# JuliaMeshless/WhatsThePoint.jl

Measured on AMD Instinct MI355X. Metric: Mpoints/sec per repel iter (k=21 KNN+force), higher is better.
Workload: dtype f32

## Files before the change

### include/wtp.h

```cpp
#ifndef WTP_H
#define WTP_H

#include <stdint.h>

#ifdef __cplusplus
extern "C" {
#endif

typedef struct wtp_ctx wtp_ctx;

typedef enum wtp_status {
    WTP_OK = 0,
    WTP_ERR_ARG = 1,
    WTP_ERR_OOM = 2,
    WTP_ERR_HIP = 3,
    WTP_ERR_STATE = 4,
    WTP_ERR_NO_DEVICE = 5
} wtp_status;

typedef enum wtp_dtype { WTP_F32 = 0, WTP_F64 = 1 } wtp_dtype;

typedef enum wtp_force_kind {
    WTP_FORCE_INVERSE_DISTANCE = 0,
    WTP_FORCE_SPACING_EQUILIBRIUM = 1,
// ... 190 lines not shown
                             double r, int64_t* d_offsets_out, wtp_block_topo_info* info);
int wtp_block_radius_fill(wtp_ctx* ctx, int64_t* d_idx_out);
int wtp_comm_exchange_peers(wtp_ctx* ctx, int n_msgs, const int* peers, const void* const* d_send, const int64_t* n_send,
                            void* const* d_recv, const int64_t* n_recv);
int wtp_comm_allgather_dev(wtp_ctx* ctx, const void* d_send, void* d_recv, int64_t bytes);

int wtp_relax_set_coverage(wtp_ctx* ctx, int axis, double lo, double hi);
int wtp_relax_set_coverage_box(wtp_ctx* ctx, const double lo[3], const double hi[3]);

int wtp_relax_set_fixed_dev(wtp_ctx* ctx, const void* d_fixed4, int64_t n_fixed_new);


int wtp_timers_get(wtp_ctx* ctx, double out[4]);
int wtp_timers_reset(wtp_ctx* ctx);
int wtp_debug_diag(wtp_ctx* ctx, unsigned long long out[16]);

int wtp_gen_uniform_dev(wtp_ctx* ctx, uint64_t seed, int64_t first, int64_t n, int dim, int dtype,
                        void* d_out);

#ifdef __cplusplus
}
#endif
#endif
```

### whatsthepoint.jl_amd/_lib.py

```python
from __future__ import annotations

import ctypes as C
import os
import subprocess

_HERE = os.path.dirname(os.path.abspath(__file__))
CSRC = os.path.join(_HERE, "csrc")
SO_PATH = os.environ.get("WTP_LIB") or os.path.join(CSRC, "libwtp.so")

WTP_OK, WTP_ERR_ARG, WTP_ERR_OOM, WTP_ERR_HIP, WTP_ERR_STATE, WTP_ERR_NO_DEVICE = range(6)
WTP_F32, WTP_F64 = 0, 1
WTP_SPACING_CONSTANT, WTP_SPACING_PER_POINT, WTP_SPACING_LOGLIKE, WTP_SPACING_BOUNDARY_LAYER = range(4)


class WtpError(RuntimeError):

    def __init__(self, code, msg):
        super().__init__(f"libwtp status {code}: {msg}")
        self.code = code


class WtpArgumentError(ValueError):
    """WTP_ERR_ARG: the reference throws ArgumentError for the same input (src/repel.jl:74)."""

# ... 102 lines not shown
    "wtp_block_step": (_i, [_vp, C.POINTER(StepStats), C.POINTER(BlockInfo)]),
    "wtp_block_run": (_i, [_vp, _i, _vp, C.POINTER(StepStats), C.POINTER(BlockInfo)]),
    "wtp_block_run_until": (_i, [_vp, _i, _d, _i, _d, _vp, C.POINTER(_i), C.POINTER(_i), C.POINTER(StepStats)]),
    "wtp_block_get": (_i, [_vp, _vp, _vp, _i64, C.POINTER(_i64)]),
    "wtp_block_close": (_i, [_vp]),
    "wtp_block_grid": (_i, [_i, C.POINTER(_i)]),
    "wtp_block_morton_rank": (_i, [_i, _i, _i, C.POINTER(_i)]),
    "wtp_block_knn": (_i, [_vp, _i, _i, _vp, _vp, _i64, _i, _i, _d, _vp, _vp, C.POINTER(BlockTopoInfo)]),
    "wtp_block_radius_offsets": (_i, [_vp, _i, _i, _vp, _vp, _i64, _d, _vp, C.POINTER(BlockTopoInfo)]),
    "wtp_block_radius_fill": (_i, [_vp, _vp]),
    "wtp_comm_exchange_peers": (_i, [_vp, _i, C.POINTER(_i), C.POINTER(_vp), C.POINTER(_i64), C.POINTER(_vp), C.POINTER(_i64)]),
    "wtp_comm_allgather_dev": (_i, [_vp, _vp, _vp, _i64]),
    "wtp_timers_get": (_i, [_vp, C.POINTER(_d)]),
    "wtp_timers_reset": (_i, [_vp]),
    "wtp_debug_diag": (_i, [_vp, C.POINTER(C.c_ulonglong)]),
    "wtp_gen_uniform_dev": (_i, [_vp, C.c_uint64, _i64, _i64, _i, _i, _vp]),
}

_lib = None


def build(verbose: bool = False) -> str:
    res = subprocess.run(["make", "-C", CSRC, "-j4"], capture_output=True, text=True)
    if res.returncode != 0:
        raise RuntimeError("building libwtp.so failed:\n" + res.stdout[-4000:] + res.stderr[-4000:])
    if verbose:
        print(res.stdout[-2000:])
    return SO_PATH


# ... 31 lines not shown
```

### whatsthepoint.jl_amd/csrc/wtp_api.hip

```cpp
#include <cmath>
#include <cstdlib>
#include <cstring>
#include <type_traits>

#include "wtp_internal.hpp"

namespace wtp {

static thread_local std::string g_create_err;

int fail(wtp_ctx* ctx, int code, const std::string& msg) {
    if (ctx)
        ctx->err = msg;
    else
        g_create_err = msg;
    return code;
}

int ensure(wtp_ctx* ctx, DevBuf& b, size_t bytes) {
    if (bytes == 0) bytes = 16;
    if (b.cap >= bytes) return WTP_OK;
    if (b.p) {
        hipFree(b.p);
        b.p = nullptr;
// ... 1172 lines not shown
    const double cell_f = (cs2 && r.spacing_kind == WTP_SPACING_CONSTANT) ? 1.01 : 1.1;
    return {cs2 ? kRhoCs2 : 3.5 * (ctx->rho / 9.0),
            cell_f * r.force.u0 * (r.spacing_typ < r.spacing_max ? r.spacing_typ : r.spacing_max)};
}

static SweepRoute step_route(const RelaxState& r, bool fresh) {
    if (!fresh) return route_ball(r.route) ? SweepRoute::Ball : SweepRoute::Exact;
    const bool measured = r.route == SweepRoute::Ksel ? r.tune.bx > 0 : !route_cs(r.route) || r.brick_hcap > 0;
    if (measured) return r.route;
    return r.route == SweepRoute::Cs64 || r.route == SweepRoute::Cs64Wave ? SweepRoute::Exact : SweepRoute::Select;
}

static int ball_pass(wtp_ctx* ctx, SearchArgs<float>& a) { return launch_cs_ball(ctx, a, a.ball_list, a.ball_count); }
static int ball_pass(wtp_ctx* ctx, SearchArgs<double>& a) { return launch_cs_ball64(ctx, a, a.ball_list, a.ball_count); }

template <typename T> static int launch_sweep(wtp_ctx* ctx, SearchArgs<T>& a, SweepRoute route, bool ball) {
    constexpr bool f32 = sizeof(T) == 4;
    ctx->n_sweep_launches += 1;
    int rc = WTP_OK, sp = -1;
    switch (route) {
    case SweepRoute::Exact:
    case SweepRoute::Ball:
        sp = span_begin(ctx, 1);
        if (route == SweepRoute::Ball) {
            rc = launch_cs_all_slots(ctx, a.fb_list, a.n, a.fb_count);
            if (!rc) rc = ball_pass(ctx, a);
        }
        if (!rc) rc = launch_generic_sweep<T>(ctx, a, route == SweepRoute::Exact);
        span_end(ctx, sp);
        return rc;
    case SweepRoute::F64Ksel:
        if constexpr (!f32) rc = relax_f64_ksel_sweep(ctx, a, &sp);
        break;
    case SweepRoute::Ksel:
        sp = span_begin(ctx, 1);
        if constexpr (f32) rc = launch_ksel_sweep(ctx, a);
        a.fb_r0 = 3;
        break;
    case SweepRoute::Select:
    case SweepRoute::Cs:
    case SweepRoute::Cs2:
        sp = span_begin(ctx, 1);
        if constexpr (f32) {
// ... 11 lines not shown
    case SweepRoute::Cs64Wave:
        sp = span_begin(ctx, 1);
        if constexpr (!f32) {
            rc = launch_brick_cs<double>(ctx, a);
            if (!rc && ball) rc = ball_pass(ctx, a);
        }
        break;
    }
    span_end(ctx, sp);
    if (rc) return rc;
    sp = span_begin(ctx, 2);
    if constexpr (f32) {
        if (route == SweepRoute::Cs2) rc = launch_cs2_followup(ctx, a);
        if (!rc && ball) rc = ball_pass(ctx, a);
    }
    if (!rc) rc = launch_generic_sweep<T>(ctx, a, false);
    span_end(ctx, sp);
    return rc;
}

template <typename T>
static HashBuild<T> relax_request(const wtp_ctx* ctx, const RelaxState& r, const Pt<T>* in, Pt<T>* out, int64_t n, int k,
                                  const HashView& view, bool keep_grid) {
    const RouteGrid g = route_grid(ctx, r);
    HashBuild<T> b(in, out, n, r.dim, k);
    b.rho_direct = g.rho;
    b.min_cell = g.min_cell;
    b.cell_scale = r.tune.scale;
    b.view = view;
    b.keep_grid = keep_grid;
    b.canonical = !r.tune.valid || r.route != SweepRoute::F64Ksel;
// ... 127 lines not shown
        a.cap_count = (float)(4.18879 * kGammaCapSweep * kGammaCapSweep * kGammaCapSweep * ctx->rho * (a.k + 1) / 22.0);
    }
    if (route == SweepRoute::Cs64 || route == SweepRoute::Cs64Wave) a.gamma_cap = (T)kGammaCap;
    a.tnn_frac = (T)kTnnFrac;
    a.cover_axis = r.cover_axis;
    a.cover_lo = (T)r.cover_lo;
    a.cover_hi = (T)r.cover_hi;
    for (int ax = 0; ax < 3; ++ax) {
        a.cover_lo3[ax] = (T)r.cover_lo3[ax];
        a.cover_hi3[ax] = (T)r.cover_hi3[ax];
    }
    a.uncovered = (int32_t*)ctx->fb_count.p + 8;
    if (!ctx->counters_clean) WTP_HIP(ctx, hipMemsetAsync(ctx->fb_count.p, 0, 64, ctx->stream));
    ctx->counters_clean = false;
    a.used_brick = a.used_wave = a.used_generic = 0;
    if ((rc = launch_sweep<T>(ctx, a, route, ball && route_ball(route)))) return rc;
    int sp = span_begin(ctx, 2);
    if (r.wall_active) {
        char* wf = (char*)ctx->wall_flags.p;
        rc = launch_mesh_constrain<T>(ctx, a.query, a.out, r.n, r.n_fixed, r.wall_offset, (const uint8_t*)wf,
                                      (uint8_t*)wf + r.wall_nm, (int32_t*)ctx->wall_tri.p, (int32_t*)ctx->wall_hint.p,
                                      (int32_t*)ctx->fb_count.p + 12);
        if (rc) return rc;
    }
    rc = launch_reduce_partials(ctx, a.partials, a.n_partials, a.used_brick, a.used_wave, a.used_generic, a.fb_count,
                                a.uncovered, r.wall_active ? (const int32_t*)ctx->fb_count.p + 12 : nullptr, d_slot);
    span_end(ctx, sp);
    if (rc) return rc;
    r.bufOld = r.bufP;
    r.bufP = o;
    r.can_revert = true;
    r.have_point_data = true;
    r.sweeps_since_rebuild += 1;
    return WTP_OK;
}

static int relax_step_any(wtp_ctx* ctx, int rebuild, wtp_step_stats* d_slot) {
    return by_dtype(ctx->relax.dtype, [&](auto t) { return relax_step_t<decltype(t)>(ctx, rebuild, d_slot); });
}
int wtp::relax_step_enqueue(wtp_ctx* ctx, int rebuild, wtp_step_stats* d_slot) { return relax_step_any(ctx, rebuild, d_slot); }

int wtp::relax_prerank(wtp_ctx* ctx, int64_t n_fixed_new) {
    RelaxState& r = ctx->relax;
// ... 722 lines not shown
    out[2] = ctx->t_other;
    out[3] = (double)ctx->n_sweep_launches;
    return WTP_OK;
}

WTP_API int wtp_timers_reset(wtp_ctx* ctx) {
    if (!ctx) return WTP_ERR_ARG;
    hipSetDevice(ctx->device);
    spans_collect(ctx);
    ctx->t_hash = ctx->t_sweep = ctx->t_other = 0;
    ctx->n_sweep_launches = 0;
    if (!ctx->timing_forced) ctx->timing = true;
    return WTP_OK;
}

WTP_API int wtp_debug_diag(wtp_ctx* ctx, unsigned long long out[16]) {
    if (!ctx || !out) return WTP_ERR_ARG;
    WTP_HIP(ctx, hipSetDevice(ctx->device));
    int rc;
    if ((rc = ensure(ctx, ctx->diag, 128))) return rc;
    WTP_HIP(ctx, hipMemcpyAsync(out, ctx->diag.p, 128, hipMemcpyDeviceToHost, ctx->stream));
    WTP_HIP(ctx, hipMemsetAsync(ctx->diag.p, 0, 128, ctx->stream));
    if ((rc = sync(ctx))) return rc;
    if (ctx->debug_kd) {
        unsigned long long kd[2] = {0, 0};
        wtp::debug_kd_steps(kd);
        fprintf(stderr, "[wtp] kd walk: %llu node visits by %llu wave-walks (%.1f per walk)\n", kd[0], kd[1], kd[1] ? (double)kd[0] / (double)kd[1] : 0.0);
    }
    return WTP_OK;
}
// ... 11 lines not shown
```

### whatsthepoint.jl_amd/csrc/wtp_device.hpp

```cpp
#pragma once
#include "wtp_internal.hpp"

namespace wtp {

template <typename T> struct Lim;
template <> struct Lim<float> {
    static __device__ __host__ constexpr float inf() { return __builtin_huge_valf(); }
};
template <> struct Lim<double> {
    static __device__ __host__ constexpr double inf() { return __builtin_huge_val(); }
};

__device__ inline float wsqrt(float x) { return __builtin_sqrtf(x); }
__device__ inline double wsqrt(double x) { return __builtin_sqrt(x); }
__device__ inline float wfloor(float x) { return floorf(x); }
__device__ inline double wfloor(double x) { return floor(x); }
__device__ inline float wpow(float a, float b) { return powf(a, b); }
__device__ inline double wpow(double a, double b) { return pow(a, b); }

template <typename T>
__device__ inline T dist2(T ax, T ay, T az, T bx, T by, T bz) {
    T dx = ax - bx;
    T dy = ay - by;
    T dz = az - bz;
// ... 182 lines not shown
    a.sum_u2 += b.sum_u2;
    a.n_move += b.n_move;
    if (b.argmin_i >= 0 &&
        (a.argmin_i < 0 || b.argmin_r < a.argmin_r || (b.argmin_r == a.argmin_r && b.argmin_i < a.argmin_i))) {
        a.argmin_r = b.argmin_r;
        a.argmin_i = b.argmin_i;
        a.argmin_j = b.argmin_j;
    }
}

__device__ inline double shfl_down_d(double v, int d) { return __shfl_down(v, d, 64); }
__device__ inline int64_t shfl_down_i64(int64_t v, int d) {
    return (int64_t)__shfl_down((long long)v, d, 64);
}

__device__ inline void acc_block_reduce(Acc& acc, Acc* smem) {
#pragma unroll
    for (int d = 32; d >= 1; d >>= 1) {
        Acc o;
        o.max_force = shfl_down_d(acc.max_force, d);
        o.sum_u = shfl_down_d(acc.sum_u, d);
        o.sum_u2 = shfl_down_d(acc.sum_u2, d);
        o.argmin_r = shfl_down_d(acc.argmin_r, d);
        o.argmin_i = shfl_down_i64(acc.argmin_i, d);
        o.argmin_j = shfl_down_i64(acc.argmin_j, d);
        o.n_move = shfl_down_i64(acc.n_move, d);
        acc_merge(acc, o);
    }
    int lane = threadIdx.x & 63, wave = threadIdx.x >> 6;
    if (lane == 0) smem[wave] = acc;
    __syncthreads();
    if (threadIdx.x == 0) {
        int nw = (blockDim.x + 63) >> 6;
        for (int w = 1; w < nw; ++w) acc_merge(acc, smem[w]);
    }
}

__device__ inline void acc_store(Partial* p, const Acc& acc) {
    p->max_force = acc.max_force;
    p->sum_u = acc.sum_u;
    p->sum_u2 = acc.sum_u2;
    p->argmin_r = acc.argmin_r;
    p->argmin_i = acc.argmin_i;
    p->argmin_j = acc.argmin_j;
    p->n_move = acc.n_move;
}

__device__ inline void reduce_partials_block(const Partial* __restrict__ parts, int n_parts, int used_brick, int wave_base,
                                             int used_wave, int used_generic, const int32_t* __restrict__ fb_count,
                                             const int32_t* __restrict__ uncovered, const int32_t* __restrict__ escaped,
                                             wtp_step_stats* __restrict__ out, int32_t* __restrict__ counters, Acc* sm) {
    Acc acc = acc_empty();
    const int total = used_brick + used_wave + used_generic;
    for (int t = threadIdx.x; t < total; t += blockDim.x) {
        const int i = t < used_brick ? t
                                     : (t < used_brick + used_wave ? wave_base + (t - used_brick)
                                                                   : n_parts - kGenericPartials + (t - used_brick - used_wave));
        if (parts[i].n_move == 0) continue;
        Acc o;
        o.max_force = parts[i].max_force;
        o.sum_u = parts[i].sum_u;
        o.sum_u2 = parts[i].sum_u2;
        o.argmin_r = parts[i].argmin_r;
        o.argmin_i = parts[i].argmin_i;
        o.argmin_j = parts[i].argmin_j;
        o.n_move = parts[i].n_move;
        acc_merge(acc, o);
    }
    acc_block_reduce(acc, sm);
    if (threadIdx.x == 0) {
        out->max_force = acc.max_force;
        out->sum_u = acc.sum_u;
        out->sum_u2 = acc.sum_u2;
        out->n_move = acc.n_move;
        out->argmin_i = acc.argmin_i;
        out->argmin_j = acc.argmin_j;
        out->argmin_r = acc.argmin_r;
        out->n_fallback = fb_count ? *fb_count : 0;
        out->n_uncovered = uncovered ? *uncovered : 0;
        out->n_escaped = escaped ? *escaped : 0;
    }
    __syncthreads();
    if (counters && threadIdx.x < 16) counters[threadIdx.x] = 0;
}


typedef float f4 __attribute__((ext_vector_type(4)));

__device__ inline uint32_t f2u(float f) { return __builtin_bit_cast(uint32_t, f); }
__device__ inline float u2f(uint32_t u) { return __builtin_bit_cast(float, u); }

__device__ inline float4 lds_pt(const void* base, uint32_t byte_off) {
    return *reinterpret_cast<const float4*>(reinterpret_cast<const unsigned char*>(base) + byte_off);
}

__device__ inline void lds_read_group(f4 (&c)[4], uint32_t addr) {
    asm volatile(
        "ds_read_b128 %0, %4\n\t"
// ... 33 lines not shown
```

### whatsthepoint.jl_amd/csrc/wtp_generic.hip

```cpp
#include "wtp_device.hpp"

namespace wtp {

static constexpr int kThreads = 128;

template <typename T, int MODE>
__global__ __launch_bounds__(kThreads) void generic_kernel(SearchArgs<T> a, const int32_t* __restrict__ list,
                                                           const int32_t* __restrict__ list_count,
                                                           int all, int part_base) {
    if (a.stop && *a.stop) return;
    __shared__ Acc sm_acc[kThreads / 64];
    const Grid<T> g = *a.grid;
    const int nq = all ? a.n : *list_count;
    const int K = a.k;
    const bool skip_self = (MODE == 0) && !a.include_self;
    T bd[kGenericKMax];
    int32_t bi[kGenericKMax];
    int32_t bp[kGenericKMax];
    Acc acc = acc_empty();

    for (int qi = blockIdx.x * blockDim.x + threadIdx.x; qi < nq; qi += gridDim.x * blockDim.x) {
        const int slot = all ? qi : list[qi];
        const Pt<T> q = a.query[slot];
        const int32_t id = w_to_id(q.w);
        if (MODE == 1 && id < a.n_fixed) {
            a.out[slot] = q;
            a.forces[slot] = (T)0;
            a.nn_dist[slot] = Lim<T>::inf();
            a.nn_id[slot] = -1;
            continue;
        }
        const int cx = cell_coord(g, q.x, 0), cy = cell_coord(g, q.y, 1), cz = cell_coord(g, q.z, 2);
        int m = 0;
        for (int r = 1;; r *= 2) {
            m = 0;
            const int z0 = cz - r < 0 ? 0 : cz - r, z1 = cz + r > g.n[2] - 1 ? g.n[2] - 1 : cz + r;
// ... 48 lines not shown
                add_force<T>(a, g.dim, s, q.x, q.y, q.z, id, c.x, c.y, c.z, bi[j], bd[j], Fx, Fy, Fz);
            }
            Pt<T> o;
            const T f = step_point<T>(a, s, q.x, q.y, q.z, Fx, Fy, Fz, o.x, o.y, o.z);
            o.w = q.w;
            a.out[slot] = o;
            a.forces[slot] = f;
            a.nn_dist[slot] = nd;
            a.nn_id[slot] = nid;
            acc_point<T>(acc, f, nd, s, id, nid);
            const T need = m == K ? bd[K - 1] : Lim<T>::inf();
            if (reaches_past_cover<T>(a, q.x, q.y, q.z, need)) atomicAdd(a.uncovered, 1);
        }
    }
    if (MODE == 1) {
        acc_block_reduce(acc, sm_acc);
        if (threadIdx.x == 0) acc_store(&a.partials[part_base + blockIdx.x], acc);
    }
}

template <typename T>
__global__ void pack_queries_kernel(const T* __restrict__ xyz, int64_t nq, int dim, Pt<T>* __restrict__ out) {
    const int64_t i = (int64_t)blockIdx.x * blockDim.x + threadIdx.x;
    if (i >= nq) return;
    Pt<T> p;
    p.x = xyz[i * dim];
    p.y = xyz[i * dim + 1];
    p.z = dim == 3 ? xyz[i * dim + 2] : (T)0;
    p.w = id_to_w((T)0, (int32_t)i);
    out[i] = p;
}

template <typename T> int launch_query_knn(wtp_ctx* ctx, SearchArgs<T>& a, const T* d_xyz, int dim, Pt<T>* d_packed) {
    hipLaunchKernelGGL(pack_queries_kernel<T>, dim3((unsigned)((a.n + 255) / 256)), dim3(256), 0, ctx->stream, d_xyz,
                       (int64_t)a.n, dim, d_packed);
    a.query = d_packed;
    a.include_self = 1;
    hipLaunchKernelGGL((generic_kernel<T, 0>), dim3(grid_for(a.n, kThreads, 4096)), dim3(kThreads), 0, ctx->stream, a,
                       (const int32_t*)nullptr, (const int32_t*)nullptr, 1, 0);
    WTP_HIP(ctx, hipGetLastError());
    return WTP_OK;
}

template <typename T>
__global__ __launch_bounds__(kThreads) void radius_kernel(SearchArgs<T> a, T r, const int64_t* __restrict__ offsets,
                                                          int32_t* __restrict__ idx_out, T* __restrict__ d2_tmp,
                                                          const int32_t* __restrict__ list,
                                                          const int32_t* __restrict__ list_count) {
    const Grid<T> g = *a.grid;
    const T r2 = r * r;
    const int nq = list ? *list_count : a.n;
    for (int qi = blockIdx.x * blockDim.x + threadIdx.x; qi < nq; qi += gridDim.x * blockDim.x) {
        const int slot = list ? list[qi] : qi;
        const Pt<T> q = a.snap[slot];
// ... 24 lines not shown
                    }
                    d2_tmp[base + pos] = d;
                    idx_out[base + pos] = cid;
                    ++m;
                }
            }
    }
}


template <typename T> int launch_generic_topology(wtp_ctx* ctx, SearchArgs<T>& a, bool all) {
    if (!a.counters_cleared) WTP_HIP(ctx, hipMemsetAsync(a.fb2_count, 0, sizeof(int32_t), ctx->stream));
    int rc = launch_wave_topology<T>(ctx, a, all);
    if (rc) return rc;
    hipLaunchKernelGGL((generic_kernel<T, 0>), dim3(256), dim3(kThreads), 0, ctx->stream, a, a.fb2_list,
                       a.fb2_count, 0, 0);
    WTP_HIP(ctx, hipGetLastError());
    return WTP_OK;
}


template <typename T> int launch_generic_sweep(wtp_ctx* ctx, SearchArgs<T>& a, bool all) {
    const int part_base = a.n_partials - kGenericPartials;
    int rc = launch_wave_sweep<T>(ctx, a, all);
    if (rc) return rc;
    a.used_generic = grid_for(a.n / 16, kThreads, 256);
    hipLaunchKernelGGL((generic_kernel<T, 1>), dim3(a.used_generic), dim3(kThreads), 0, ctx->stream, a, a.fb2_list,
                       a.fb2_count, 0, part_base);
    WTP_HIP(ctx, hipGetLastError());
    return WTP_OK;
}

template <typename T> static bool brick_radius_usable(wtp_ctx*, SearchArgs<T>&) { return false; }
template <> bool brick_radius_usable<float>(wtp_ctx* ctx, SearchArgs<float>& a) {
    return !ctx->force_generic && a.fb_list != nullptr && a.fb_count != nullptr;
}
template <typename T> static int brick_radius(wtp_ctx*, SearchArgs<T>&) { return WTP_OK; }
template <> int brick_radius<float>(wtp_ctx* ctx, SearchArgs<float>& a) { return launch_brick_radius(ctx, a); }

__global__ void radius_copy_rows_kernel(int64_t n, const int32_t* __restrict__ tmp, const uint8_t* __restrict__ done,
                                        const int32_t* __restrict__ arena, const int64_t* __restrict__ arena_off,
                                        const int64_t* __restrict__ offsets, int32_t* __restrict__ idx) {
    const int64_t grp = ((int64_t)blockIdx.x * blockDim.x + threadIdx.x) >> 4, ngrp = ((int64_t)gridDim.x * blockDim.x) >> 4;
// ... 67 lines not shown
    int rc;
    if ((brick_radius_usable<T>(ctx, a) && a.rad_tmp) || a.rad_dense)
        rc = launch_wave_radius_fill<T>(ctx, a, r, d_offsets, d_idx, a.fb_list, a.fb_count);
    else
        rc = launch_wave_radius_fill<T>(ctx, a, r, d_offsets, d_idx, nullptr, nullptr);
    if (rc) return rc;
    hipLaunchKernelGGL((radius_kernel<T>), dim3(256), dim3(kThreads), 0, ctx->stream, a, r, d_offsets, d_idx,
                       (T*)ctx->scratch.p, (const int32_t*)a.fb2_list, (const int32_t*)a.fb2_count);
    WTP_HIP(ctx, hipGetLastError());
    return WTP_OK;
}

#define INST(T)                                                                              \
    template int launch_generic_topology<T>(wtp_ctx*, SearchArgs<T>&, bool);                 \
    template int launch_query_knn<T>(wtp_ctx*, SearchArgs<T>&, const T*, int, Pt<T>*);         \
    template int launch_generic_sweep<T>(wtp_ctx*, SearchArgs<T>&, bool);                    \
    template int launch_radius_count<T>(wtp_ctx*, SearchArgs<T>&, T, int32_t*);              \
    template int launch_radius_fill<T>(wtp_ctx*, SearchArgs<T>&, T, const int64_t*, int32_t*);
INST(float)
INST(double)
#undef INST

}
```

### whatsthepoint.jl_amd/csrc/wtp_hash.hip

```cpp
#include "wtp_device.hpp"

namespace wtp {

static constexpr int kThreads = 256;

template <typename T>
__global__ void load_points_kernel(const T* __restrict__ xyz, Pt<T>* __restrict__ out, int64_t n, int dim) {
    int64_t i = (int64_t)blockIdx.x * blockDim.x + threadIdx.x;
    int64_t stride = (int64_t)gridDim.x * blockDim.x;
    for (; i < n; i += stride) {
        Pt<T> p;
        p.x = xyz[i * dim + 0];
        p.y = xyz[i * dim + 1];
        p.z = dim == 3 ? xyz[i * dim + 2] : (T)0;
        p.w = id_to_w((T)0, (int32_t)i);
        out[i] = p;
    }
}

template <typename T>
__global__ void bbox_kernel(const Pt<T>* __restrict__ pts, int64_t n, T* __restrict__ part, int64_t v_old = 0,
                            int32_t v_fixed_old = 0) {
    __shared__ T sm[6][kThreads / 64];
    T mn[3] = {Lim<T>::inf(), Lim<T>::inf(), Lim<T>::inf()};
// ... 798 lines not shown
    for (; i < n; i += stride)
        for (int a = 0; a < dim; ++a) {
            uint64_t h = splitmix64((seed << 40) + 3ull * (uint64_t)(first + i) + (uint64_t)a);
            out[i * dim + a] = (T)((float)(h >> 40) * (1.0f / 16777216.0f));
        }
}

template <typename T>
int launch_gen_uniform(wtp_ctx* ctx, uint64_t seed, int64_t first, int64_t n, int dim, T* d_out) {
    hipLaunchKernelGGL(gen_uniform_kernel<T>, dim3(grid_for(n, kThreads, 8192)), dim3(kThreads), 0,
                       ctx->stream, seed, first, n, dim, d_out);
    WTP_HIP(ctx, hipGetLastError());
    return WTP_OK;
}

__global__ void reduce_partials_kernel(const Partial* __restrict__ parts, int n_parts, int used_brick, int wave_base,
                                       int used_wave, int used_generic, const int32_t* __restrict__ fb_count,
                                       const int32_t* __restrict__ uncovered, const int32_t* __restrict__ escaped,
                                       wtp_step_stats* __restrict__ out, int32_t* __restrict__ counters) {
    __shared__ Acc sm[kThreads / 64];
    reduce_partials_block(parts, n_parts, used_brick, wave_base, used_wave, used_generic, fb_count, uncovered, escaped, out,
                          counters, sm);
}

int launch_reduce_partials(wtp_ctx* ctx, const Partial* parts, int n_parts, int used_brick, int used_wave,
                           int used_generic, const int32_t* fb_count, const int32_t* uncovered, const int32_t* escaped,
                           wtp_step_stats* d_slot) {
    hipLaunchKernelGGL(reduce_partials_kernel, dim3(1), dim3(kThreads), 0, ctx->stream, parts, n_parts, used_brick,
                       brick_partials(), used_wave, used_generic, fb_count, uncovered, escaped, d_slot,
                       (int32_t*)ctx->fb_count.p);
    ctx->counters_clean = true;
    WTP_HIP(ctx, hipGetLastError());
    return WTP_OK;
}

static constexpr int kLayerPasses = 32;
static constexpr int kLayerChunk = kThreads * kLayerPasses;

int layer_blocks(int64_t n) { return (int)((n + kLayerChunk - 1) / kLayerChunk); }

template <typename T> __device__ inline T axis_of(const Pt<T>& p, int axis) {
    return axis == 0 ? p.x : (axis == 1 ? p.y : p.z);
}

__device__ inline int64_t layer_slot(int block, int wave, int pass, int lane) {
// ... 253 lines not shown
```

### whatsthepoint.jl_amd/csrc/wtp_internal.hpp

```cpp
#pragma once
#include <hip/hip_runtime.h>
#include <stdint.h>
#include <map>
#include <string>
#include <utility>
#include <vector>

#include "../../include/wtp.h"

namespace wtp {

template <typename T> struct PtOf;
template <> struct PtOf<float> { using type = float4; };
template <> struct PtOf<double> { using type = double4; };
template <typename T> using Pt = typename PtOf<T>::type;

template <typename F> inline auto by_dtype(int dtype, F&& f) { return dtype == WTP_F32 ? f(float{}) : f(double{}); }

__host__ __device__ inline float id_to_w(float, int32_t id) { return __builtin_bit_cast(float, id); }
__host__ __device__ inline double id_to_w(double, int32_t id) {
    return __builtin_bit_cast(double, (int64_t)id);
}
__host__ __device__ inline int32_t w_to_id(float w) { return __builtin_bit_cast(int32_t, w); }
__host__ __device__ inline int32_t w_to_id(double w) {
// ... 31 lines not shown
constexpr double kGammaCapSweep = 0.96;
constexpr double kTnnFrac = 0.8;
constexpr double kRhoCs2 = 1.0;
constexpr double kRhoKsel = 1.2;
constexpr double kCapKsel = 40.0;
constexpr int kGridReuseMax = 7;

struct Partial {
    double max_force;
    double sum_u;
    double sum_u2;
    double argmin_r;
    int64_t argmin_i;
    int64_t argmin_j;
    int64_t n_move;
};

struct ForceParams {
    int32_t kind;
    double beta, u0, gamma;
};

template <typename T> struct SearchArgs {
    const Grid<T>* grid;
    const Pt<T>* snap;
    const int32_t* cell_start;
    const Pt<T>* query;
    int32_t n;
    int32_t k;
    int32_t include_self;
// ... 191 lines not shown
    size_t cs2_smem = 0;
    const void* cs2_fn = nullptr;
    int cs2_occ = 0;
    std::map<std::pair<const void*, size_t>, int> launch_cache;
    wtp::GridTune knn_tune, knn64_tune;
    wtp::DevBuf pts[3];
    wtp::DevBuf raw_in;
    wtp::DevBuf cell_of, rank_of, cell_cnt, cell_start, scan_tmp;
    wtp::DevBuf grid, bbox_part, occ;
    wtp::DevBuf box_dev;
    wtp::DevBuf idx_out, dist_out, counts_out;
    wtp::DevBuf cand_idx, cand_dist, f32_pts;
    wtp::DevBuf grid_b, cell_start_b, box_b, f64k_s64, f64k_slot, f64k_lists, f64k_cnt;
    wtp::DevBuf forces, nn_dist, nn_id, spacing_pp;
    wtp::DevBuf partials, stats, fb_list, fb_count, fb2_list, fb2_count, nn_list;
    wtp::DevBuf rad_pos;
    wtp::DevBuf rad_bricks;
    bool rad_dense_attr[2] = {false, false};
    bool rad_dense_used = false;
    wtp::DevBuf rad_tmp, rad_done;
    wtp::DevBuf rad_arena, rad_arena_off;
    wtp::DevBuf brick_dead;
    wtp::Prerank prerank;
    int64_t preranked_builds = 0;
    hipStream_t comm_stream = nullptr;
    hipEvent_t ev_comm_a = nullptr, ev_comm_b = nullptr;
    bool hash_scratch_clean = false;
    bool counters_clean = false;
    wtp::DevBuf stop_state;
    const int32_t* stop_dev = nullptr;
// ... 83 lines not shown
    return (int)(b > cap ? cap : b);
}
template <typename T> int launch_topology(wtp_ctx* ctx, SearchArgs<T>& a);
int launch_brick_sweep(wtp_ctx* ctx, SearchArgs<float>& a, bool cs);
template <typename T> int launch_brick_cs(wtp_ctx* ctx, SearchArgs<T>& a);
template <typename T> int launch_wave_topology(wtp_ctx* ctx, SearchArgs<T>& a, bool all);
template <typename T> int launch_wave_sweep(wtp_ctx* ctx, SearchArgs<T>& a, bool all);
template <typename T>
int launch_wave_radius_count(wtp_ctx* ctx, SearchArgs<T>& a, T r, int32_t* d_counts, const int32_t* list,
                             const int32_t* list_count);
template <typename T>
int launch_wave_radius_fill(wtp_ctx* ctx, SearchArgs<T>& a, T r, const int64_t* d_offsets, int32_t* d_idx,
                            const int32_t* list, const int32_t* list_count);
template <typename T> int launch_generic_topology(wtp_ctx* ctx, SearchArgs<T>& a, bool all);
template <typename T> int launch_query_knn(wtp_ctx* ctx, SearchArgs<T>& a, const T* d_xyz, int dim, Pt<T>* d_packed);
template <typename T> int launch_generic_sweep(wtp_ctx* ctx, SearchArgs<T>& a, bool all);
inline int total_partials() { return brick_partials() + kWavePartials + kGenericPartials; }
int launch_brick_radius(wtp_ctx* ctx, SearchArgs<float>& a);
int launch_cs2(wtp_ctx* ctx, SearchArgs<float>& a);
int launch_cs2_followup(wtp_ctx* ctx, SearchArgs<float>& a);
int debug_kd_steps(unsigned long long out[2]);
int launch_cs_ball(wtp_ctx* ctx, SearchArgs<float>& a, int32_t* rest_list, int32_t* rest_count);
int launch_cs2_census(wtp_ctx* ctx, int BX, unsigned int* d_out513);
int launch_cs2_dead(wtp_ctx* ctx, SearchArgs<float>& a, uint8_t* d_dead, int dead_cap);
int cs2_max_bx();
int launch_ksel_topology(wtp_ctx* ctx, SearchArgs<float>& a);
int launch_ksel_sweep(wtp_ctx* ctx, SearchArgs<float>& a);
int ksel_max_bx();
int ksel_kmax();
template <typename T>
int launch_radius_count(wtp_ctx* ctx, SearchArgs<T>& a, T r, int32_t* d_counts);
template <typename T>
int launch_radius_fill(wtp_ctx* ctx, SearchArgs<T>& a, T r, const int64_t* d_offsets,
                       int32_t* d_idx);
int launch_reduce_partials(wtp_ctx* ctx, const Partial* parts, int n_parts, int used_brick, int used_wave,
                           int used_generic, const int32_t* fb_count, const int32_t* uncovered,
                           const int32_t* escaped, wtp_step_stats* d_stats_slot);
template <typename T>
int launch_pca_normals(wtp_ctx* ctx, const T* d_xyz, int64_t n, int dim, const int32_t* d_rows, int k, T* d_out);
template <typename T>
int launch_minplus_batch(wtp_ctx* ctx, const int32_t* d_rows, const T* d_dist, int64_t n, int k, double g, double tol,
                         T* d_h0, T* d_h1, int first, int sweeps, unsigned long long* d_state);
template <typename TP>
int launch_mesh_constrain(wtp_ctx* ctx, const Pt<TP>* old, Pt<TP>* cur, int64_t n, int64_t n_fixed, double offset,
                          const uint8_t* is_bnd, uint8_t* escaped, int32_t* tri_idx, int32_t* hint, int32_t* n_escaped);
template <typename T>
int launch_unpermute(wtp_ctx* ctx, const Pt<T>* pts, int64_t n, int64_t n_fixed, int dim, T* d_xyz_out);
template <typename T>
int launch_unpermute_point_data(wtp_ctx* ctx, const Pt<T>* pts, int64_t n, int64_t n_fixed,
                                const T* forces, const T* nn_dist, const int32_t* nn_id,
                                T* forces_o, T* nn_dist_o, int32_t* nn_id_o);
template <typename T>
// ... 67 lines not shown
```

### whatsthepoint.jl_amd/csrc/wtp_wave.hip

```cpp
#include "wtp_device.hpp"

namespace wtp {

static constexpr int kWaves = 4;
static constexpr int kThreads = kWaves * 64;
static constexpr int kCap = 512;
static constexpr int kKeyRegs = kCap / 64;
static constexpr int kSurv = 256;

template <typename T> struct Bits;
template <> struct Bits<float> {
    using U = uint32_t;
    static __device__ U of(float v) { return __builtin_bit_cast(uint32_t, v); }
    static __device__ float back(U u) { return __builtin_bit_cast(float, u); }
    static constexpr U kInf = 0x7F800000u;
};
template <> struct Bits<double> {
    using U = uint64_t;
    static __device__ U of(double v) { return __builtin_bit_cast(uint64_t, v); }
    static __device__ double back(U u) { return __builtin_bit_cast(double, u); }
    static constexpr U kInf = 0x7FF0000000000000ull;
};

template <typename T, bool SWEEP> struct WaveSmem;
// ... 22 lines not shown

template <typename T, int MODE>
__global__ __launch_bounds__(kThreads) void wave_kernel(SearchArgs<T> a, const int32_t* __restrict__ list,
                                                        const int32_t* __restrict__ list_count, int all,
                                                        int part_base) {
    if (a.stop && *a.stop) return;
    extern __shared__ __attribute__((aligned(16))) unsigned char smem_raw[];
    using U = typename Bits<T>::U;
    const int wave = threadIdx.x >> 6;
    const int lane = threadIdx.x & 63;
    using Smem = WaveSmem<T, MODE == 1>;
    Smem* sm = reinterpret_cast<Smem*>(smem_raw) + wave;
    Acc* sm_acc = reinterpret_cast<Acc*>(smem_raw + sizeof(Smem) * kWaves);
    const Grid<T> g = *a.grid;
    const int nq = all ? a.n : *list_count;
    const int K = a.k;
    const bool skip_self = (MODE == 0) && !a.include_self;
    Acc acc = acc_empty();
    const int wave_global = blockIdx.x * kWaves + wave;
    const int wave_stride = gridDim.x * kWaves;

    for (int qi = wave_global; qi < nq; qi += wave_stride) {
        const int slot = all ? qi : list[qi];
        const Pt<T> q = a.query[slot];
        const int32_t id = w_to_id(q.w);
        if (MODE == 1 && id < a.n_fixed) {
            if (lane == 0) {
                a.out[slot] = q;
                a.forces[slot] = (T)0;
                a.nn_dist[slot] = Lim<T>::inf();
// ... 491 lines not shown
```

Measured before the change: 12510.

## Fuse step-stat reduction into generic sweep kernel via last-block completion

```diff
diff --git a/include/wtp.h b/include/wtp.h
--- a/include/wtp.h
+++ b/include/wtp.h
@@ -228,6 +228,7 @@
 int wtp_timers_get(wtp_ctx* ctx, double out[4]);
 int wtp_timers_reset(wtp_ctx* ctx);
 int wtp_debug_diag(wtp_ctx* ctx, unsigned long long out[16]);
+int wtp_debug_counters(wtp_ctx* ctx, int32_t out[16]);
 
 int wtp_gen_uniform_dev(wtp_ctx* ctx, uint64_t seed, int64_t first, int64_t n, int dim, int dtype,
                         void* d_out);
diff --git a/whatsthepoint.jl_amd/_lib.py b/whatsthepoint.jl_amd/_lib.py
--- a/whatsthepoint.jl_amd/_lib.py
+++ b/whatsthepoint.jl_amd/_lib.py
@@ -140,6 +140,7 @@
     "wtp_timers_get": (_i, [_vp, C.POINTER(_d)]),
     "wtp_timers_reset": (_i, [_vp]),
     "wtp_debug_diag": (_i, [_vp, C.POINTER(C.c_ulonglong)]),
+    "wtp_debug_counters": (_i, [_vp, C.POINTER(C.c_int32)]),
     "wtp_gen_uniform_dev": (_i, [_vp, C.c_uint64, _i64, _i64, _i, _i, _vp]),
 }
 
diff --git a/whatsthepoint.jl_amd/csrc/wtp_api.hip b/whatsthepoint.jl_amd/csrc/wtp_api.hip
--- a/whatsthepoint.jl_amd/csrc/wtp_api.hip
+++ b/whatsthepoint.jl_amd/csrc/wtp_api.hip
@@ -1210,7 +1210,7 @@
 static int ball_pass(wtp_ctx* ctx, SearchArgs<float>& a) { return launch_cs_ball(ctx, a, a.ball_list, a.ball_count); }
 static int ball_pass(wtp_ctx* ctx, SearchArgs<double>& a) { return launch_cs_ball64(ctx, a, a.ball_list, a.ball_count); }
 
-template <typename T> static int launch_sweep(wtp_ctx* ctx, SearchArgs<T>& a, SweepRoute route, bool ball) {
+template <typename T> static int launch_sweep(wtp_ctx* ctx, SearchArgs<T>& a, SweepRoute route, bool ball, StepReduce* red) {
     constexpr bool f32 = sizeof(T) == 4;
     ctx->n_sweep_launches += 1;
     int rc = WTP_OK, sp = -1;
@@ -1222,7 +1222,7 @@
             rc = launch_cs_all_slots(ctx, a.fb_list, a.n, a.fb_count);
             if (!rc) rc = ball_pass(ctx, a);
         }
-        if (!rc) rc = launch_generic_sweep<T>(ctx, a, route == SweepRoute::Exact);
+        if (!rc) rc = launch_generic_sweep<T>(ctx, a, route == SweepRoute::Exact, red);
         span_end(ctx, sp);
         return rc;
     case SweepRoute::F64Ksel:
@@ -1264,7 +1264,7 @@
         if (route == SweepRoute::Cs2) rc = launch_cs2_followup(ctx, a);
         if (!rc && ball) rc = ball_pass(ctx, a);
     }
-    if (!rc) rc = launch_generic_sweep<T>(ctx, a, false);
+    if (!rc) rc = launch_generic_sweep<T>(ctx, a, false, red);
     span_end(ctx, sp);
     return rc;
 }
@@ -1422,19 +1422,30 @@
     if (!ctx->counters_clean) WTP_HIP(ctx, hipMemsetAsync(ctx->fb_count.p, 0, 64, ctx->stream));
     ctx->counters_clean = false;
     a.used_brick = a.used_wave = a.used_generic = 0;
-    if ((rc = launch_sweep<T>(ctx, a, route, ball && route_ball(route)))) return rc;
-    int sp = span_begin(ctx, 2);
+    if ((rc = ensure(ctx, ctx->last_counters, 64))) return rc;
+    StepReduce red{};
+    red.parts = a.partials;
+    red.n_parts = a.n_partials;
+    red.wave_base = brick_partials();
+    red.uncovered = a.uncovered;
+    red.counters = (int32_t*)ctx->fb_count.p;
+    red.last_counters = (int32_t*)ctx->last_counters.p;
+    red.out = r.wall_active ? nullptr : d_slot;
+    if ((rc = launch_sweep<T>(ctx, a, route, ball && route_ball(route), &red))) return rc;
     if (r.wall_active) {
+        int sp = span_begin(ctx, 2);
         char* wf = (char*)ctx->wall_flags.p;
         rc = launch_mesh_constrain<T>(ctx, a.query, a.out, r.n, r.n_fixed, r.wall_offset, (const uint8_t*)wf,
                                       (uint8_t*)wf + r.wall_nm, (int32_t*)ctx->wall_tri.p, (int32_t*)ctx->wall_hint.p,
                                       (int32_t*)ctx->fb_count.p + 12);
         if (rc) return rc;
-    }
-    rc = launch_reduce_partials(ctx, a.partials, a.n_partials, a.used_brick, a.used_wave, a.used_generic, a.fb_count,
-                                a.uncovered, r.wall_active ? (const int32_t*)ctx->fb_count.p + 12 : nullptr, d_slot);
-    span_end(ctx, sp);
-    if (rc) return rc;
+        red.escaped = (const int32_t*)ctx->fb_count.p + 12;
+        red.out = d_slot;
+        rc = launch_reduce_partials(ctx, red);
+        span_end(ctx, sp);
+        if (rc) return rc;
+    }
+    ctx->counters_clean = true;
     r.bufOld = r.bufP;
     r.bufP = o;
     r.can_revert = true;
@@ -2187,6 +2198,16 @@
     return WTP_OK;
 }
 
+WTP_API int wtp_debug_counters(wtp_ctx* ctx, int32_t out[16]) {
+    if (!ctx || !out) return WTP_ERR_ARG;
+    WTP_HIP(ctx, hipSetDevice(ctx->device));
+    int rc;
+    if ((rc = sync(ctx))) return rc;
+    memset(out, 0, 16 * sizeof(int32_t));
+    if (ctx->last_counters.p) WTP_HIP(ctx, hipMemcpy(out, ctx->last_counters.p, 16 * sizeof(int32_t), hipMemcpyDeviceToHost));
+    return WTP_OK;
+}
+
 WTP_API int wtp_debug_diag(wtp_ctx* ctx, unsigned long long out[16]) {
     if (!ctx || !out) return WTP_ERR_ARG;
     WTP_HIP(ctx, hipSetDevice(ctx->device));
diff --git a/whatsthepoint.jl_amd/csrc/wtp_device.hpp b/whatsthepoint.jl_amd/csrc/wtp_device.hpp
--- a/whatsthepoint.jl_amd/csrc/wtp_device.hpp
+++ b/whatsthepoint.jl_amd/csrc/wtp_device.hpp
@@ -220,7 +220,7 @@
     return (int64_t)__shfl_down((long long)v, d, 64);
 }
 
-__device__ inline void acc_block_reduce(Acc& acc, Acc* smem) {
+__device__ inline void acc_wave_reduce(Acc& acc) {
 #pragma unroll
     for (int d = 32; d >= 1; d >>= 1) {
         Acc o;
@@ -233,6 +233,9 @@
         o.n_move = shfl_down_i64(acc.n_move, d);
         acc_merge(acc, o);
     }
+}
+__device__ inline void acc_block_reduce(Acc& acc, Acc* smem) {
+    acc_wave_reduce(acc);
     int lane = threadIdx.x & 63, wave = threadIdx.x >> 6;
     if (lane == 0) smem[wave] = acc;
     __syncthreads();
@@ -252,29 +255,54 @@
     p->n_move = acc.n_move;
 }
 
-__device__ inline void reduce_partials_block(const Partial* __restrict__ parts, int n_parts, int used_brick, int wave_base,
-                                             int used_wave, int used_generic, const int32_t* __restrict__ fb_count,
-                                             const int32_t* __restrict__ uncovered, const int32_t* __restrict__ escaped,
-                                             wtp_step_stats* __restrict__ out, int32_t* __restrict__ counters, Acc* sm) {
-    Acc acc = acc_empty();
-    const int total = used_brick + used_wave + used_generic;
-    for (int t = threadIdx.x; t < total; t += blockDim.x) {
-        const int i = t < used_brick ? t
-                                     : (t < used_brick + used_wave ? wave_base + (t - used_brick)
-                                                                   : n_parts - kGenericPartials + (t - used_brick - used_wave));
-        if (parts[i].n_move == 0) continue;
-        Acc o;
-        o.max_force = parts[i].max_force;
-        o.sum_u = parts[i].sum_u;
-        o.sum_u2 = parts[i].sum_u2;
-        o.argmin_r = parts[i].argmin_r;
-        o.argmin_i = parts[i].argmin_i;
-        o.argmin_j = parts[i].argmin_j;
-        o.n_move = parts[i].n_move;
-        acc_merge(acc, o);
-    }
-    acc_block_reduce(acc, sm);
+constexpr int kReduceThreads = 256;
+template <int NT> __device__ inline void reduce_partials_block(const StepReduce& r, Acc* sm ) {
+    static_assert(kReduceThreads % NT == 0 && NT % 64 == 0, "the block must tile the reduction's threads in whole waves");
+    constexpr int V = kReduceThreads / NT;
+    const int nw = r.wave_count ? (__hip_atomic_load(r.wave_count, __ATOMIC_RELAXED, __HIP_MEMORY_SCOPE_AGENT) +
+                                   kWaveQueriesPerBlock - 1) / kWaveQueriesPerBlock
+                                : r.used_wave;
+    const int ng = r.generic_count ? (__hip_atomic_load(r.generic_count, __ATOMIC_RELAXED, __HIP_MEMORY_SCOPE_AGENT) +
+                                      kGenericQueriesPerBlock - 1) / kGenericQueriesPerBlock
+                                   : r.used_generic;
+    const int used_wave = nw < r.used_wave ? nw : r.used_wave, used_generic = ng < r.used_generic ? ng : r.used_generic;
+    const int total = r.used_brick + used_wave + used_generic;
+#pragma unroll
+    for (int v = 0; v < V; ++v) {
+        Acc acc = acc_empty();
+        for (int t0 = threadIdx.x + v * NT; t0 < total; t0 += 4 * kReduceThreads) {
+            Partial q[4];
+#pragma unroll
+            for (int u = 0; u < 4; ++u) {
+                const int t = t0 + u * kReduceThreads;
+                const int i = t < r.used_brick ? t
+                                               : (t < r.used_brick + used_wave ? r.wave_base + (t - r.used_brick)
+                                                                                 : r.n_parts - kGenericPartials + (t - r.used_brick - used_wave));
+                if (t < total) q[u] = r.parts[i];
+                else q[u].n_move = 0;
+            }
+#pragma unroll
+            for (int u = 0; u < 4; ++u) {
+                if (q[u].n_move == 0) continue;
+                Acc o;
+                o.max_force = q[u].max_force;
+                o.sum_u = q[u].sum_u;
+                o.sum_u2 = q[u].sum_u2;
+                o.argmin_r = q[u].argmin_r;
+                o.argmin_i = q[u].argmin_i;
+                o.argmin_j = q[u].argmin_j;
+                o.n_move = q[u].n_move;
+                acc_merge(acc, o);
+            }
+        }
+        acc_wave_reduce(acc);
+        if ((threadIdx.x & 63) == 0) sm[(threadIdx.x + v * NT) >> 6] = acc;
+    }
+    __syncthreads();
     if (threadIdx.x == 0) {
+        Acc acc = sm[0];
+        for (int w = 1; w < kReduceThreads / 64; ++w) acc_merge(acc, sm[w]);
+        wtp_step_stats* out = r.out;
         out->max_force = acc.max_force;
         out->sum_u = acc.sum_u;
         out->sum_u2 = acc.sum_u2;
@@ -282,12 +310,31 @@
         out->argmin_i = acc.argmin_i;
         out->argmin_j = acc.argmin_j;
         out->argmin_r = acc.argmin_r;
-        out->n_fallback = fb_count ? *fb_count : 0;
-        out->n_uncovered = uncovered ? *uncovered : 0;
-        out->n_escaped = escaped ? *escaped : 0;
-    }
-    __syncthreads();
-    if (counters && threadIdx.x < 16) counters[threadIdx.x] = 0;
+        out->n_fallback = r.fb_count ? __hip_atomic_load(r.fb_count, __ATOMIC_RELAXED, __HIP_MEMORY_SCOPE_AGENT) : 0;
+        out->n_uncovered = r.uncovered ? __hip_atomic_load(r.uncovered, __ATOMIC_RELAXED, __HIP_MEMORY_SCOPE_AGENT) : 0;
+        out->n_escaped = r.escaped ? __hip_atomic_load(r.escaped, __ATOMIC_RELAXED, __HIP_MEMORY_SCOPE_AGENT) : 0;
+    }
+    __syncthreads();
+    if (r.counters && threadIdx.x < 16) {
+        const int32_t c = __hip_atomic_load(r.counters + threadIdx.x, __ATOMIC_RELAXED, __HIP_MEMORY_SCOPE_AGENT);
+        if (r.last_counters) r.last_counters[threadIdx.x] = c;
+        r.counters[threadIdx.x] = 0;
+    }
+}
+
+template <int NT> __device__ inline void finish_step(const StepReduce& r, Acc* sm ) {
+    __shared__ int last;
+    __syncthreads();
+    if (threadIdx.x == 0) {
+        __builtin_amdgcn_fence(__ATOMIC_RELEASE, "agent");
+        last = atomicAdd(r.counters + 15, 1) == (int)gridDim.x - 1;
+        __builtin_amdgcn_fence(__ATOMIC_ACQUIRE, "agent");
+    }
+    __syncthreads();
+    if (last) {
+        __builtin_amdgcn_fence(__ATOMIC_ACQUIRE, "agent");
+        reduce_partials_block<NT>(r, sm);
+    }
 }
 
 
diff --git a/whatsthepoint.jl_amd/csrc/wtp_generic.hip b/whatsthepoint.jl_amd/csrc/wtp_generic.hip
--- a/whatsthepoint.jl_amd/csrc/wtp_generic.hip
+++ b/whatsthepoint.jl_amd/csrc/wtp_generic.hip
@@ -3,15 +3,17 @@
 namespace wtp {
 
 static constexpr int kThreads = 128;
+static_assert(kThreads == kGenericQueriesPerBlock, "the step's reduction sizes the serial kernel's slots by kGenericQueriesPerBlock");
 
 template <typename T, int MODE>
 __global__ __launch_bounds__(kThreads) void generic_kernel(SearchArgs<T> a, const int32_t* __restrict__ list,
                                                            const int32_t* __restrict__ list_count,
-                                                           int all, int part_base) {
+                                                           int all, int part_base, StepReduce red) {
     if (a.stop && *a.stop) return;
-    __shared__ Acc sm_acc[kThreads / 64];
+    __shared__ Acc sm_acc[kReduceThreads / 64];
     const Grid<T> g = *a.grid;
     const int nq = all ? a.n : *list_count;
+    const bool idle = MODE == 1 && !all && (int)blockIdx.x * kThreads >= nq;
     const int K = a.k;
     const bool skip_self = (MODE == 0) && !a.include_self;
     T bd[kGenericKMax];
@@ -19,7 +21,7 @@
     int32_t bp[kGenericKMax];
     Acc acc = acc_empty();
 
-    for (int qi = blockIdx.x * blockDim.x + threadIdx.x; qi < nq; qi += gridDim.x * blockDim.x) {
+    for (int qi = blockIdx.x * blockDim.x + threadIdx.x; !idle && qi < nq; qi += gridDim.x * blockDim.x) {
         const int slot = all ? qi : list[qi];
         const Pt<T> q = a.query[slot];
         const int32_t id = w_to_id(q.w);
@@ -98,8 +100,11 @@
         }
     }
     if (MODE == 1) {
-        acc_block_reduce(acc, sm_acc);
-        if (threadIdx.x == 0) acc_store(&a.partials[part_base + blockIdx.x], acc);
+        if (!idle) {
+            acc_block_reduce(acc, sm_acc);
+            if (threadIdx.x == 0) acc_store(&a.partials[part_base + blockIdx.x], acc);
+        }
+        if (red.out) finish_step<kThreads>(red, sm_acc);
     }
 }
 
@@ -121,7 +126,7 @@
     a.query = d_packed;
     a.include_self = 1;
     hipLaunchKernelGGL((generic_kernel<T, 0>), dim3(grid_for(a.n, kThreads, 4096)), dim3(kThreads), 0, ctx->stream, a,
-                       (const int32_t*)nullptr, (const int32_t*)nullptr, 1, 0);
+                       (const int32_t*)nullptr, (const int32_t*)nullptr, 1, 0, StepReduce{});
     WTP_HIP(ctx, hipGetLastError());
     return WTP_OK;
 }
@@ -176,19 +181,26 @@
     int rc = launch_wave_topology<T>(ctx, a, all);
     if (rc) return rc;
     hipLaunchKernelGGL((generic_kernel<T, 0>), dim3(256), dim3(kThreads), 0, ctx->stream, a, a.fb2_list,
-                       a.fb2_count, 0, 0);
+                       a.fb2_count, 0, 0, StepReduce{});
     WTP_HIP(ctx, hipGetLastError());
     return WTP_OK;
 }
 
 
-template <typename T> int launch_generic_sweep(wtp_ctx* ctx, SearchArgs<T>& a, bool all) {
+template <typename T> int launch_generic_sweep(wtp_ctx* ctx, SearchArgs<T>& a, bool all, StepReduce* finish) {
     const int part_base = a.n_partials - kGenericPartials;
+    const int32_t* wave_count = all ? nullptr : a.fb_count;
     int rc = launch_wave_sweep<T>(ctx, a, all);
     if (rc) return rc;
     a.used_generic = grid_for(a.n / 16, kThreads, 256);
+    finish->used_brick = a.used_brick;
+    finish->used_wave = a.used_wave;
+    finish->used_generic = a.used_generic;
+    finish->wave_count = wave_count;
+    finish->generic_count = a.fb2_count;
+    finish->fb_count = a.fb_count;
     hipLaunchKernelGGL((generic_kernel<T, 1>), dim3(a.used_generic), dim3(kThreads), 0, ctx->stream, a, a.fb2_list,
-                       a.fb2_count, 0, part_base);
+                       a.fb2_count, 0, part_base, *finish);
     WTP_HIP(ctx, hipGetLastError());
     return WTP_OK;
 }
@@ -286,7 +298,7 @@
 #define INST(T)                                                                              \
     template int launch_generic_topology<T>(wtp_ctx*, SearchArgs<T>&, bool);                 \
     template int launch_query_knn<T>(wtp_ctx*, SearchArgs<T>&, const T*, int, Pt<T>*);         \
-    template int launch_generic_sweep<T>(wtp_ctx*, SearchArgs<T>&, bool);                    \
+    template int launch_generic_sweep<T>(wtp_ctx*, SearchArgs<T>&, bool, StepReduce*);                    \
     template int launch_radius_count<T>(wtp_ctx*, SearchArgs<T>&, T, int32_t*);              \
     template int launch_radius_fill<T>(wtp_ctx*, SearchArgs<T>&, T, const int64_t*, int32_t*);
 INST(float)
diff --git a/whatsthepoint.jl_amd/csrc/wtp_hash.hip b/whatsthepoint.jl_amd/csrc/wtp_hash.hip
--- a/whatsthepoint.jl_amd/csrc/wtp_hash.hip
+++ b/whatsthepoint.jl_amd/csrc/wtp_hash.hip
@@ -836,21 +836,13 @@
     return WTP_OK;
 }
 
-__global__ void reduce_partials_kernel(const Partial* __restrict__ parts, int n_parts, int used_brick, int wave_base,
-                                       int used_wave, int used_generic, const int32_t* __restrict__ fb_count,
-                                       const int32_t* __restrict__ uncovered, const int32_t* __restrict__ escaped,
-                                       wtp_step_stats* __restrict__ out, int32_t* __restrict__ counters) {
-    __shared__ Acc sm[kThreads / 64];
-    reduce_partials_block(parts, n_parts, used_brick, wave_base, used_wave, used_generic, fb_count, uncovered, escaped, out,
-                          counters, sm);
-}
-
-int launch_reduce_partials(wtp_ctx* ctx, const Partial* parts, int n_parts, int used_brick, int used_wave,
-                           int used_generic, const int32_t* fb_count, const int32_t* uncovered, const int32_t* escaped,
-                           wtp_step_stats* d_slot) {
-    hipLaunchKernelGGL(reduce_partials_kernel, dim3(1), dim3(kThreads), 0, ctx->stream, parts, n_parts, used_brick,
-                       brick_partials(), used_wave, used_generic, fb_count, uncovered, escaped, d_slot,
-                       (int32_t*)ctx->fb_count.p);
+__global__ void reduce_partials_kernel(StepReduce r) {
+    __shared__ Acc sm[kReduceThreads / 64];
+    reduce_partials_block<kThreads>(r, sm);
+}
+
+int launch_reduce_partials(wtp_ctx* ctx, const StepReduce& red) {
+    hipLaunchKernelGGL(reduce_partials_kernel, dim3(1), dim3(kThreads), 0, ctx->stream, red);
     ctx->counters_clean = true;
     WTP_HIP(ctx, hipGetLastError());
     return WTP_OK;
diff --git a/whatsthepoint.jl_amd/csrc/wtp_internal.hpp b/whatsthepoint.jl_amd/csrc/wtp_internal.hpp
--- a/whatsthepoint.jl_amd/csrc/wtp_internal.hpp
+++ b/whatsthepoint.jl_amd/csrc/wtp_internal.hpp
@@ -69,6 +69,21 @@
     int64_t argmin_i;
     int64_t argmin_j;
     int64_t n_move;
+};
+
+constexpr int kWaveQueriesPerBlock = 4;
+constexpr int kGenericQueriesPerBlock = 128;
+struct StepReduce {
+    const Partial* parts;
+    int32_t n_parts, used_brick, wave_base, used_wave, used_generic;
+    const int32_t* wave_count;
+    const int32_t* generic_count;
+    const int32_t* fb_count;
+    const int32_t* uncovered;
+    const int32_t* escaped;
+    wtp_step_stats* out;
+    int32_t* counters;
+    int32_t* last_counters;
 };
 
 struct ForceParams {
@@ -290,6 +305,7 @@
     wtp::DevBuf grid_b, cell_start_b, box_b, f64k_s64, f64k_slot, f64k_lists, f64k_cnt;
     wtp::DevBuf forces, nn_dist, nn_id, spacing_pp;
     wtp::DevBuf partials, stats, fb_list, fb_count, fb2_list, fb2_count, nn_list;
+    wtp::DevBuf last_counters;
     wtp::DevBuf rad_pos;
     wtp::DevBuf rad_bricks;
     bool rad_dense_attr[2] = {false, false};
@@ -403,7 +419,7 @@
                             const int32_t* list, const int32_t* list_count);
 template <typename T> int launch_generic_topology(wtp_ctx* ctx, SearchArgs<T>& a, bool all);
 template <typename T> int launch_query_knn(wtp_ctx* ctx, SearchArgs<T>& a, const T* d_xyz, int dim, Pt<T>* d_packed);
-template <typename T> int launch_generic_sweep(wtp_ctx* ctx, SearchArgs<T>& a, bool all);
+template <typename T> int launch_generic_sweep(wtp_ctx* ctx, SearchArgs<T>& a, bool all, StepReduce* finish);
 inline int total_partials() { return brick_partials() + kWavePartials + kGenericPartials; }
 int launch_brick_radius(wtp_ctx* ctx, SearchArgs<float>& a);
 int launch_cs2(wtp_ctx* ctx, SearchArgs<float>& a);
@@ -422,9 +438,7 @@
 template <typename T>
 int launch_radius_fill(wtp_ctx* ctx, SearchArgs<T>& a, T r, const int64_t* d_offsets,
                        int32_t* d_idx);
-int launch_reduce_partials(wtp_ctx* ctx, const Partial* parts, int n_parts, int used_brick, int used_wave,
-                           int used_generic, const int32_t* fb_count, const int32_t* uncovered,
-                           const int32_t* escaped, wtp_step_stats* d_stats_slot);
+int launch_reduce_partials(wtp_ctx* ctx, const StepReduce& red);
 template <typename T>
 int launch_pca_normals(wtp_ctx* ctx, const T* d_xyz, int64_t n, int dim, const int32_t* d_rows, int k, T* d_out);
 template <typename T>
diff --git a/whatsthepoint.jl_amd/csrc/wtp_wave.hip b/whatsthepoint.jl_amd/csrc/wtp_wave.hip
--- a/whatsthepoint.jl_amd/csrc/wtp_wave.hip
+++ b/whatsthepoint.jl_amd/csrc/wtp_wave.hip
@@ -4,6 +4,7 @@
 
 static constexpr int kWaves = 4;
 static constexpr int kThreads = kWaves * 64;
+static_assert(kWaves == kWaveQueriesPerBlock, "the step's reduction sizes the wave kernel's slots by kWaveQueriesPerBlock");
 static constexpr int kCap = 512;
 static constexpr int kKeyRegs = kCap / 64;
 static constexpr int kSurv = 256;
@@ -60,6 +61,7 @@
     Acc* sm_acc = reinterpret_cast<Acc*>(smem_raw + sizeof(Smem) * kWaves);
     const Grid<T> g = *a.grid;
     const int nq = all ? a.n : *list_count;
+    if (MODE == 1 && !all && (int)blockIdx.x * kWaves >= nq) return;
     const int K = a.k;
     const bool skip_self = (MODE == 0) && !a.include_self;
     Acc acc = acc_empty();
```

Result: faster. 12820, median of 6 (+2.4%).
